# cvxgrp/pymde

Measured on AMD Instinct MI355X. Metric: edges/sec/iter (avg_distortion fwd+bwd), n=1M |E|=50M d=2, higher is better.
Workload: dtype f32; 1 GPU; BASELINE configs[3] / SURVEY 8d config 4a: n=1000000, |E|=50000000 uniform-random edges (out-degree 50), d=2, penalties.Log1p(1.5), weights in {1,2}; seeded on the device with torch.Generator(0) (the survey's recipe uses numpy default_rng(0): same distribution, another stream; --survey-seed builds that one); parallelism=single GPU, parameter_stream=codebook: 2 distinct weights ride in the packed half-edge word (4 B/half-edge)

## Files before the change

### include/mde_hip.h

```cpp
#ifndef MDE_HIP_H_
#define MDE_HIP_H_

#include <stdint.h>

#ifdef __cplusplus
extern "C" {
#endif

#define MDE_ABI_VERSION 2

#define MDE_OK 0
#define MDE_E_INVALID (-1)
#define MDE_E_SELF_EDGE (-2)
#define MDE_E_RANGE (-3)
#define MDE_E_TOO_LARGE (-4)
#define MDE_E_HIP (-5)
#define MDE_E_UNSUPPORTED (-6)

const char* mde_last_error(void);
int mde_abi_version(void);

enum {
  MDE_F_NONE = 0,
  MDE_F_LINEAR = 1,
// ... 59 lines not shown
int mde_shard_bounds(int64_t n, int64_t p, const int64_t* edges, int32_t world,
                     int64_t* bounds_host, void* stream);

int mde_plan_expand(const mde_plan* plan, const float* in_edge, float* out_half, void* stream);

int mde_plan_layout(mde_plan* plan, int32_t d, void* stream);
int mde_plan_function_hint(mde_plan* plan, int32_t kind, int32_t kind_neg);
int64_t mde_plan_layout_half_edges(const mde_plan* plan, int32_t layout);
int mde_plan_expand_codebook(const mde_plan* plan, const float* in_edge, float* out_half,
                             int32_t* n_values_host, void* stream);
int mde_plan_expand_bytes(const mde_plan* plan, const float* in_edge, float* out_half,
                          int32_t* n_values_host, void* stream);
int mde_plan_expand_layout(const mde_plan* plan, int32_t layout, const float* in_edge,
                           float* out_half, void* stream);
int mde_plan_ring_info(const mde_plan* plan, int64_t* info_host);
int mde_plan_ring_check(const mde_plan* plan, int64_t* out_host, void* stream);
int mde_plan_row_order(mde_plan* plan, int32_t mode, void* stream, double* info_host);
int mde_plan_loss_double(const mde_plan* plan, double* dst, void* stream);

int mde_edges_deduplicate(int64_t n, int64_t p, const int64_t* edges, int64_t* edges_out,
                          int64_t* count_host, void* stream);
int mde_edges_count_unique(int64_t n, int64_t p, const int64_t* edges, int64_t* edges_out,
                           float* weights_out, int64_t* count_host, void* stream);
int mde_knn(int64_t n, int32_t nf, const float* data, int32_t k, int32_t* idx_out, float* d2_out,
            float* sqn_work, void* stream);
int mde_row_sqnorm(int64_t n, int32_t nf, const float* data, float* out, void* stream);
int64_t mde_col_stats_work_bytes(int64_t n, int32_t nf);
int mde_col_stats(int64_t n, int32_t nf, const float* data, double* stats_out, int32_t* bad_row_out, void* work,
                  void* stream);
int mde_rows_subtract(int64_t n, int32_t nf, const float* data, const double* mu, float* out, void* stream);
// ... 193 lines not shown
```

### pymde_amd/_lib.py

```python
import ctypes
import os
import threading

import torch

_HERE = os.path.dirname(os.path.abspath(__file__))
LIB_PATH = os.path.join(_HERE, "libmde_hip.so")

c_i32, c_i64, c_f32 = ctypes.c_int32, ctypes.c_int64, ctypes.c_float
c_vp = ctypes.c_void_p

MDE_OK = 0
MDE_E_INVALID, MDE_E_SELF_EDGE, MDE_E_RANGE = -1, -2, -3
MDE_E_TOO_LARGE, MDE_E_HIP, MDE_E_UNSUPPORTED = -4, -5, -6


class MdeFunc(ctypes.Structure):
    _fields_ = [("kind", c_i32), ("kind_neg", c_i32), ("a0", c_vp), ("a1", c_vp),
                ("a0_scalar", c_i32), ("a1_scalar", c_i32),
                ("s0", c_f32), ("s1", c_f32), ("s2", c_f32),
                ("n0", c_f32), ("n1", c_f32), ("n2", c_f32), ("layout", c_i32),
                ("e0", c_vp), ("e1", c_vp)]


# ... 13 lines not shown
    "mde_plan_destroy": (c_i32, [c_vp]),
    "mde_plan_n": (c_i64, [c_vp]),
    "mde_plan_p": (c_i64, [c_vp]),
    "mde_plan_half_edges": (c_i64, [c_vp]),
    "mde_plan_row_lo": (c_i64, [c_vp]),
    "mde_plan_row_hi": (c_i64, [c_vp]),
    "mde_plan_rowptr": (c_vp, [c_vp]),
    "mde_plan_nbr": (c_vp, [c_vp]),
    "mde_plan_eid": (c_vp, [c_vp]),
    "mde_plan_export": (c_i32, [c_vp, c_vp, c_vp, c_vp, c_vp]),
    "mde_shard_bounds": (c_i32, [c_i64, c_i64, c_vp, c_i32, ctypes.POINTER(c_i64), c_vp]),
    "mde_plan_expand": (c_i32, [c_vp, c_vp, c_vp, c_vp]),
    "mde_plan_layout": (c_i32, [c_vp, c_i32, c_vp]),
    "mde_plan_layout_half_edges": (c_i64, [c_vp, c_i32]),
    "mde_plan_ring_info": (c_i32, [c_vp, ctypes.POINTER(c_i64)]),
    "mde_plan_ring_check": (c_i32, [c_vp, ctypes.POINTER(c_i64), c_vp]),
    "mde_plan_row_order": (c_i32, [c_vp, c_i32, c_vp, ctypes.POINTER(ctypes.c_double)]),
    "mde_plan_function_hint": (c_i32, [c_vp, c_i32, c_i32]),
    "mde_plan_loss_double": (c_i32, [c_vp, c_vp, c_vp]),
    "mde_center_step_begin": (c_i32, [c_i64, c_i32, c_vp, c_vp, c_f32, c_vp, c_vp, c_vp]),
    "mde_center_step_end": (c_i32, [c_i64, c_i32, c_vp, c_vp, ctypes.c_double, c_vp]),
    "mde_lbfgs_dev_stage": (c_i32, [c_vp, c_vp, c_vp, c_vp, c_f32, c_vp, c_vp]),
    "mde_lbfgs_dev_finish": (c_i32, [c_vp, c_vp, c_vp, c_vp, c_vp, c_vp]),
    "mde_lbfgs_dev_dots": (c_i32, [c_vp]),
    "mde_rank_reduce": (c_i32, [c_i32, c_i32, ctypes.c_uint64, c_vp, c_vp, c_i32, c_vp, c_vp]),
    "mde_plan_expand_codebook": (c_i32, [c_vp, c_vp, c_vp, ctypes.POINTER(c_i32), c_vp]),
    "mde_plan_expand_bytes": (c_i32, [c_vp, c_vp, c_vp, ctypes.POINTER(c_i32), c_vp]),
    "mde_plan_expand_layout": (c_i32, [c_vp, c_i32, c_vp, c_vp, c_vp]),
    "mde_edges_deduplicate": (c_i32, [c_i64, c_i64, c_vp, c_vp, ctypes.POINTER(c_i64), c_vp]),
    "mde_edges_count_unique": (c_i32, [c_i64, c_i64, c_vp, c_vp, c_vp, ctypes.POINTER(c_i64), c_vp]),
# ... 161 lines not shown
```

### pymde_amd/average_distortion.py

```python
import ctypes

import torch

from pymde_amd import _lib
from pymde_amd import util


def _check_X(X, n=None, d=None):
    if not isinstance(X, torch.Tensor) or X.dim() != 2:
        raise ValueError("the embedding must be a 2-D tensor")
    if X.dtype != torch.float32:
        raise ValueError(
            "pymde_amd computes in float32; got an embedding of dtype %s (MDE.embed and "
            "MDE.average_distortion cast float64 inputs with a warning; the kernels themselves do not)" % X.dtype)
    util.require_cuda_device(X.device)
    if n is not None and X.shape[0] != n:
        raise ValueError("embedding has %d rows, the problem has %d items" % (X.shape[0], n))


class EdgePlan(object):

    def __init__(self, n_items, edges, row_lo=0, row_hi=None):
        lib = _lib.load()
        device = util.require_cuda_device(edges.device)
# ... 61 lines not shown
        if t.numel() != self.p:
            return None
        size = int(lib.mde_plan_layout_half_edges(self._handle, 1))
        out = torch.empty(max(size, 1), dtype=torch.float32, device=self.device)
        nv = ctypes.c_int32(0)
        with torch.cuda.device(self.device):
            _lib.check(lib.mde_plan_expand_bytes(self._handle, _lib.ptr(t), _lib.ptr(out),
                                                 ctypes.byref(nv), _lib.stream_ptr(self.device)))
        return out if nv.value > 0 else None

    def ring_info(self):
        lib = _lib.load()
        info = (ctypes.c_int64 * 16)()
        _lib.check(lib.mde_plan_ring_info(self._handle, info))
        names = ("built", "d", "rows_per_block", "row_blocks", "col_groups", "chunks", "ring_slots", "iterations",
                 "ring_half_edges", "padded_entries", "permuted", "hub_rows", "hub_half_edges", "hub_segments")
        out = {k: int(info[i]) for i, k in enumerate(names)}
        out["built"], out["permuted"] = bool(out["built"]), bool(out["permuted"])
        return out

    def ring_check(self):
        lib = _lib.load()
        out = (ctypes.c_int64 * 3)()
        with torch.cuda.device(self.device):
            _lib.check(lib.mde_plan_ring_check(self._handle, out, _lib.stream_ptr(self.device)))
        return {"split": int(out[0]), "shared": int(out[1]), "pairs": int(out[2])}

    def row_order(self, mode=1):
        lib = _lib.load()
        info = (ctypes.c_double * 4)()
        with torch.cuda.device(self.device):
            _lib.check(lib.mde_plan_row_order(self._handle, int(mode), _lib.stream_ptr(self.device), info))
        return {"in_use": bool(info[0]), "mean_distance_before": float(info[1]),
                "mean_distance_after": float(info[2]), "levels": int(info[3])}

    def csr(self):
        lib = _lib.load()
        nloc = self.row_hi - self.row_lo
        rowptr = torch.empty(nloc + 1, dtype=torch.int32, device=self.device)
        nbr = torch.empty(max(self.half_edges, 1), dtype=torch.int32, device=self.device)
        eid = torch.empty(max(self.half_edges, 1), dtype=torch.int32, device=self.device)
# ... 224 lines not shown
```

### pymde_amd/csrc/mde_plan.h

```cpp
#pragma once
#include "mde_common.h"

struct mde_ring_layout {
  int d = 0;
  int rejected_d = 0;
  float cost_scale = 1.0f;
  int rows_per_block = 0, n_row_blocks = 0;
  int col_groups = 1;
  int chunk_cols = 0, n_chunks = 0;
  int ring_off = 0, slots = 0;
  int64_t n_iters = 0;
  int64_t H = 0;
  uint32_t* packed = nullptr;
  int32_t* eid = nullptr;
  uint32_t* hdr = nullptr;
  int32_t* wave_iter = nullptr;
  float* partial = nullptr;
  int32_t* slot_row = nullptr;
  int count_all = 0;
  int n_hub_rows = 0, n_hub_segs = 0;
  int64_t hub_half_edges = 0;
  int32_t* hub_rows = nullptr;
  int32_t* hub_seg = nullptr;
  int32_t* hub_first = nullptr;
  double* hub_partial = nullptr;
};
#define MDE_HUB_SEG 512

struct mde_plan {
  int64_t n = 0, p = 0, H = 0, row_lo = 0, row_hi = 0;
  int32_t* rowptr = nullptr;
  int32_t* nbr = nullptr;
  int32_t* eid = nullptr;
  double* partials = nullptr;
// ... 22 lines not shown
```

### pymde_amd/csrc/mde_ring.h

```cpp
#pragma once
#include "mde_common.h"
#include "mde_functions.h"
#include "mde_plan.h"

#define MDE_RING_LDS_BYTES 163840
__host__ __device__ constexpr int ring_row_cap(int d) { return d == 1 ? 12288 : (d == 2 ? 7816 : (d == 3 ? 5200 : 3936)); }
__host__ __device__ constexpr int ring_ctrl_off(int d) { return (ring_row_cap(d) + 32) * 4 * d; }
__host__ __device__ constexpr int ring_gr_off(int d) { return ring_ctrl_off(d) + 256; }
#define MDE_RING_CTRL_PROG(d) (ring_ctrl_off(d))
#define MDE_RING_CTRL_F(d) (ring_ctrl_off(d) + 64)
#define MDE_RING_CTRL_CB(d) (ring_ctrl_off(d) + 96)
#ifndef MDE_RING_NCW
#define MDE_RING_NCW 8
#endif
#ifndef MDE_RING_CSLEEP
#define MDE_RING_CSLEEP 1
#endif
#ifndef MDE_RING_PSLEEP
#define MDE_RING_PSLEEP 1
#endif
#ifndef MDE_RING_PRODPRIO
#define MDE_RING_PRODPRIO 2
#endif
#ifndef MDE_RING_CONSPRIO
// ... 39 lines not shown
#ifdef MDE_RING_SPAN
  return MDE_RING_SPAN;
#endif
  return S - 5 > 6 ? 6 : (S - 5 < 2 ? 2 : S - 5);
}

#define MDE_RING_HDR(m, span, rounds, pad) ((uint32_t)(m) | ((uint32_t)(span) << 16) | ((uint32_t)(rounds) << 21) | ((uint32_t)(pad) << 27))

#define MDE_RING_HW 4
#define MDE_RING_H3_PAD 4u

__host__ __device__ inline uint32_t ring_pack_word(int d, uint32_t rowaddr, uint32_t coladdr) {
  return d == 2 ? (rowaddr | ((coladdr >> 3) << 16)) : (rowaddr | ((coladdr >> 2) << 16));
}

struct RingArgs {
  mde_plan* plan;
  const float* X;
  int d;
  const float *a0, *a1;
  int a0_scalar, a1_scalar;
  float* grad;
  float inv_p, grad_scale;
  hipStream_t st;
  float* loss_out;
  double loss_scale;
};

inline MdeFuncArgs ring_func_args(const mde_func* f) {
  MdeFuncArgs a;
// ... 15 lines not shown
```

### pymde_amd/csrc/mde_ring.hip

```cpp
#include <algorithm>
#include <chrono>
#include <cmath>
#include <cstring>
#include <vector>

#include "mde_ring.h"

#ifndef MDE_RING_BUCKETS
#define MDE_RING_BUCKETS 32
#endif
__global__ __launch_bounds__(64) void k_ring_assign(int nloc, int R, int Q, int NC, int C, int contiguous,
                                                    const int32_t* __restrict__ rowptr,
                                                    const int32_t* __restrict__ nbr, uint32_t* __restrict__ wmap,
                                                    int32_t* __restrict__ wrows) {
  constexpr int B = MDE_RING_BUCKETS, NCWP = MDE_RING_NCW <= 8 ? 8 : 16, LPW = 64 / NCWP, BPL = B / LPW;
  static_assert(MDE_RING_NCW <= 16 && B % LPW == 0 && B <= 64, "lane map of k_ring_assign");
  __shared__ int hist[B];
  __shared__ float cpre[B];
  const int wg = blockIdx.x, rb = wg / Q, g = wg % Q, lane = threadIdx.x;
  const int j_lo = (int)(((int64_t)g * NC + Q - 1) / Q), j_hi = (int)(((int64_t)(g + 1) * NC + Q - 1) / Q);
  const int nj = max(1, j_hi - j_lo);
  const int r0 = rb * R, nr = min(R, nloc - r0);
  const int w = lane / LPW, bg = lane % LPW;
  uint32_t* out = wmap + (size_t)wg * R;
// ... 378 lines not shown
  }
  return half * 32 + quarter * 16 + pos;
}

__global__ __launch_bounds__(MDE_BLOCK) void k_ring_pack(int64_t nit, int nseg, const int32_t* __restrict__ iter_base,
                                                         const int32_t* __restrict__ src_base,
                                                         const int32_t* __restrict__ it_ent,
                                                         const int32_t* __restrict__ it_cnt,
                                                         const int32_t* __restrict__ it_m,
                                                         const uint32_t* __restrict__ keys,
                                                         const uint32_t* __restrict__ vals,
                                                         const int32_t* __restrict__ hrow,
                                                         const int32_t* __restrict__ nbr,
                                                         const int32_t* __restrict__ eid, int R, int Q, int C, int S,
                                                         int ring_off, int JB, int d, int row_lo, int place, int count_all,
                                                         uint32_t* __restrict__ packed,
                                                         int32_t* __restrict__ peid, uint32_t* __restrict__ hdr) {
  __shared__ uint8_t s_taken[MDE_BLOCK / 64][64], s_free[MDE_BLOCK / 64][64];
  __shared__ uint32_t s_prow[MDE_BLOCK / 64][64];
  const int lane = threadIdx.x & 63, wv = threadIdx.x >> 6;
  const int64_t nw = ((int64_t)gridDim.x * MDE_BLOCK) >> 6;
  const uint32_t JM = (1u << JB) - 1u;
  const int sh = ring_cls_shift(d), cm = ring_cls_mask(d);
  const uint32_t cbytes = (uint32_t)C * 4u * (uint32_t)d;
  for (int64_t itb = (int64_t)blockIdx.x * (MDE_BLOCK / 64); itb < nit; itb += nw) {
    const int64_t it = itb + wv;
    const bool valid = it < nit;
    int64_t src = it;
    if (valid && src_base) {
      int lo = 0, hi = nseg;
      while (hi - lo > 1) {
// ... 46 lines not shown
      }
    }
    __syncthreads();
    const bool moved = second && act && pin < 0 && s_taken[wv][l];
    if (second && act && !moved) s_taken[wv][l] = 1;
    __syncthreads();
    {
      const bool fr = !s_taken[wv][lane];
      const unsigned long long fm = __ballot(fr);
      if (fr) s_free[wv][__popcll(fm & ((1ull << lane) - 1ull))] = (uint8_t)lane;
    }
    __syncthreads();
    const unsigned long long mvm = __ballot(moved);
    const int nmoved = __popcll(mvm);
    if (moved) l = s_free[wv][__popcll(mvm & ((1ull << lane) - 1ull))];
    const bool counts = act && (count_all || (uint32_t)(row_lo + grow) < col);
    const int ncount = __popcll(__ballot(counts));
    const uint32_t lclass = ncount == 0 ? 0u : (ncount == cnt ? 1u : 2u);
    const uint32_t m = valid ? (uint32_t)__builtin_amdgcn_readfirstlane(it_m[src]) : 0u;
    const uint32_t need = max((uint32_t)(cw >> 8), m);
    const uint32_t mpad = valid ? (uint32_t)__builtin_amdgcn_readfirstlane(it_m[src & ~(int64_t)1]) : 0u;
    const size_t base = ((size_t)(it >> 2) * 64) * 4 + (size_t)(it & 3);
    if (act) {
      packed[base + (size_t)l * 4] = ring_pack_word(d, rowaddr, ring);
      peid[base + (size_t)l * 4] = eid[q];
    } else if (valid) {
      const int lf = s_free[wv][nmoved + lane - cnt];
      packed[base + (size_t)lf * 4] = ring_pack_word(d, (uint32_t)(R + (lf & 31)) * 4u * (uint32_t)d,
                                                     (uint32_t)ring_off + (mpad % (uint32_t)S) * cbytes);
      peid[base + (size_t)lf * 4] = -1;
    }
    if (lane == 0 && valid) {
      hdr[MDE_RING_HW * it] = m;
      hdr[MDE_RING_HW * it + 1] = need;
      hdr[MDE_RING_HW * it + 2] = lclass;
      hdr[MDE_RING_HW * it + 3] = (cnt < 64 ? MDE_RING_H3_PAD : 0u) | ((uint32_t)cnt << 8);
    }
    __syncthreads();
  }
}

__global__ __launch_bounds__(MDE_BLOCK) void k_ring_block_class(int64_t nblocks, uint32_t* __restrict__ hdr) {
  const int64_t b = (int64_t)blockIdx.x * MDE_BLOCK + threadIdx.x;
  if (b >= nblocks) return;
  bool any0 = false, any1 = false, any2 = false;
  for (int q = 0; q < 4; ++q) {
    const uint32_t* h = hdr + (size_t)MDE_RING_HW * (4 * b + q);
    if ((h[3] >> 8) == 0u) continue;
    any0 |= h[2] == 0u;
    any1 |= h[2] == 1u;
    any2 |= h[2] == 2u;
// ... 13 lines not shown
__global__ __launch_bounds__(MDE_BLOCK) void k_ring_stats(int64_t nit, const uint32_t* __restrict__ hdr,
                                                          unsigned long long* __restrict__ stats) {
  unsigned long long a = 0, b = 0, c = 0;
  for (int64_t i = (int64_t)blockIdx.x * MDE_BLOCK + threadIdx.x; i < nit; i += (int64_t)gridDim.x * MDE_BLOCK) {
    a += (hdr[MDE_RING_HW * i + 3] & MDE_RING_H3_PAD) ? 1u : 0u;
    b += hdr[MDE_RING_HW * i + 2] == 1u;
    c += hdr[MDE_RING_HW * i + 2] == 2u;
  }
  a = mde_wave_sum(a);
  b = mde_wave_sum(b);
  c = mde_wave_sum(c);
  if ((threadIdx.x & 63) == 0) {
    atomicAdd(&stats[0], a);
    atomicAdd(&stats[1], b);
    atomicAdd(&stats[2], c);
  }
}

__global__ __launch_bounds__(MDE_BLOCK) void k_ring_sweep_balance(int nwg, int ngroups, int GW, int JB,
                                                                  const uint32_t* __restrict__ keys,
                                                                  const int32_t* __restrict__ seg,
                                                                  unsigned long long* __restrict__ crit,
                                                                  unsigned long long* __restrict__ tot) {
  const int64_t idx = (int64_t)blockIdx.x * MDE_BLOCK + threadIdx.x;
  if (idx >= (int64_t)nwg * ngroups) return;
  const int wg = (int)(idx / ngroups), g = (int)(idx % ngroups);
  unsigned long long mx = 0, sm = 0;
  for (int w = 0; w < MDE_RING_NCW; ++w) {
    const uint32_t s = (uint32_t)wg * MDE_RING_NCW + (uint32_t)w;
    const int32_t lo = seg[s], hi = seg[s + 1];
// ... 574 lines not shown
  if (e == hipSuccess) e = hipMalloc(&peid, (size_t)Hp * sizeof(int32_t));
  if (e == hipSuccess) e = hipMalloc(&hdr, (size_t)total_iters * MDE_RING_HW * sizeof(uint32_t));
  const size_t partial_floats = (size_t)z.Q * (size_t)nloc * (size_t)d;
  if (e == hipSuccess && z.Q > 1) e = hipMalloc(&partial, sizeof(float) * (partial_floats + 2 * (size_t)z.NRB));
  if (e == hipSuccess && z.Q > 1) e = hipMemsetAsync(partial + partial_floats, 0, sizeof(float) * 2 * (size_t)z.NRB, st);
  if (e != hipSuccess) {
    drop_caps();
    return fail(e, "ring layout: output allocations");
  }
  tick("output allocations");
  if (!single) {
    hipLaunchKernelGGL(k_ring_schedule<true>, dim3(nseg), dim3(64), flag_bytes, st, nseg, seg, wrows, keys2, meta, JM, span, z.R,
                       z.Q, z.NC, d, cap, 0, nullptr, iter_base, it_ent, it_cnt, it_m, flag_rows, nullptr);
    e = hipGetLastError();
  }
  if (e == hipSuccess) {
    hipLaunchKernelGGL(k_ring_pack, dim3(mde_grid((int64_t)total_iters * 64, MDE_BLOCK, 8192)), dim3(MDE_BLOCK), 0, st,
                       (int64_t)total_iters, nseg, iter_base, single ? cap_base : nullptr, it_ent, it_cnt, it_m, keys2, vals2, hrow,
                       plan->nbr, plan->eid, z.R, z.Q, z.C, z.S, z.ring_off, z.JB, d, (int)plan->row_lo, place, rp.permuted ? 1 : 0,
                       packed, peid, hdr);
    e = hipGetLastError();
  }
  if (e == hipSuccess) e = hipStreamSynchronize(st);
  drop_caps();
  if (e != hipSuccess) return fail(e, "ring layout: fill / pack");
  hipLaunchKernelGGL(k_ring_block_class, dim3((unsigned)((total_iters / 4 + MDE_BLOCK - 1) / MDE_BLOCK)), dim3(MDE_BLOCK), 0, st,
                     (int64_t)(total_iters / 4), hdr);
  RB(hipGetLastError());
  RB(hipStreamSynchronize(st));
  if (getenv("MDE_RING_STATS")) {
    unsigned long long* dstat = reinterpret_cast<unsigned long long*>(iters);
    unsigned long long hstat[3] = {0, 0, 0};
    RB(hipMemsetAsync(dstat, 0, sizeof(hstat), st));
    hipLaunchKernelGGL(k_ring_stats, dim3(256), dim3(MDE_BLOCK), 0, st, (int64_t)total_iters, hdr, dstat);
    RB(hipMemcpyAsync(hstat, dstat, sizeof(hstat), hipMemcpyDeviceToHost, st));
    RB(hipStreamSynchronize(st));
    {
      std::vector<int32_t> hb((size_t)nseg + 1);
      RB(hipMemcpy(hb.data(), iter_base, hb.size() * sizeof(int32_t), hipMemcpyDeviceToHost));
      int mx = 0, mn = 1 << 30, wg_mx = 0;
      for (int i = 0; i < nseg; ++i) {
        mx = std::max(mx, hb[i + 1] - hb[i]);
        mn = std::min(mn, hb[i + 1] - hb[i]);
      }
// ... 63 lines not shown
  L.n_row_blocks = z.NRB;
  L.col_groups = z.Q;
  L.chunk_cols = z.C;
  L.n_chunks = z.NC;
  L.ring_off = z.ring_off;
  L.slots = z.S;
  L.n_iters = total_iters;
  L.H = Hp;
  L.packed = packed;
  L.eid = peid;
  L.hdr = hdr;
  L.wave_iter = iter_base;
  L.partial = partial;
  L.slot_row = slot_row;
  L.count_all = rp.permuted ? 1 : 0;
  L.n_hub_rows = (int)rp.hub_rows.size();
  L.n_hub_segs = (int)(rp.hub_seg.size() / 4);
  L.hub_half_edges = rp.hub_half_edges;
  L.hub_rows = hub_rows;
  L.hub_seg = hub_seg;
  L.hub_first = hub_first;
  L.hub_partial = hub_partial;
  return 1;
}

extern "C" int mde_plan_layout(mde_plan* plan, int32_t d, void* stream) {
  if (!plan || d <= 0) return MDE_E_INVALID;
  if (plan->ring.packed && plan->ring.d == d) return 1;
  RingSizes z;
  if (!choose_sizes(plan, d, &z)) return 0;
// ... 292 lines not shown
  if (!L.packed) return MDE_OK;
  info[0] = 1;
  info[1] = L.d;
  info[2] = L.rows_per_block;
  info[3] = L.n_row_blocks;
  info[4] = L.col_groups;
  info[5] = L.n_chunks;
  info[6] = L.slots;
  info[7] = L.n_iters;
  info[8] = plan->H - L.hub_half_edges;
  info[9] = L.H;
  info[10] = L.slot_row ? 1 : 0;
  info[11] = L.n_hub_rows;
  info[12] = L.hub_half_edges;
  info[13] = L.n_hub_segs;
  return MDE_OK;
}

__global__ __launch_bounds__(MDE_BLOCK) void k_ring_pair_check(int64_t npairs, const uint32_t* __restrict__ packed, int d, int R,
                                                               unsigned long long* __restrict__ out) {
  const int lane = threadIdx.x & 63;
  const int64_t nw = ((int64_t)gridDim.x * MDE_BLOCK) >> 6;
  const uint32_t mask = d == 2 ? 0xfff8u : 0xfffcu, dummy = (uint32_t)R * 4u * (uint32_t)d;
  unsigned long long split = 0, shared = 0, pairs = 0;
  for (int64_t pr = ((int64_t)blockIdx.x * MDE_BLOCK + threadIdx.x) >> 6; pr < npairs; pr += nw) {
    const int64_t it = 2 * pr;
    const size_t base = ((size_t)(it >> 2) * 64 + (size_t)lane) * 4 + (size_t)(it & 3);
    const uint32_t ra = packed[base] & mask, rb = packed[base + 1] & mask;
    int found = -1;
    for (int k = 0; k < 64; ++k)
      if ((uint32_t)__builtin_amdgcn_readlane((int)ra, k) == rb) found = k;
    const bool real = rb < dummy;
    split += __popcll(__ballot(real && found >= 0 && found != lane));
    shared += __popcll(__ballot(real && found >= 0));
    ++pairs;
  }
  if (lane == 0) {
    atomicAdd(&out[0], split);
    atomicAdd(&out[1], shared);
    atomicAdd(&out[2], pairs);
  }
}

extern "C" int mde_plan_ring_check(const mde_plan* plan, int64_t* out_host, void* stream) {
  if (!plan || !out_host) return MDE_E_INVALID;
  const mde_ring_layout& L = plan->ring;
  for (int i = 0; i < 3; ++i) out_host[i] = 0;
  if (!L.packed || L.n_iters == 0) return MDE_OK;
  hipStream_t st = mde_stream(stream);
  unsigned long long* dout = nullptr;
  hipError_t e = hipMalloc(&dout, 3 * sizeof(unsigned long long));
  if (e == hipSuccess) e = hipMemsetAsync(dout, 0, 3 * sizeof(unsigned long long), st);
  if (e == hipSuccess) {
    hipLaunchKernelGGL(k_ring_pair_check, dim3(mde_grid(L.n_iters / 2 * 64, MDE_BLOCK, 4096)), dim3(MDE_BLOCK), 0, st,
                       L.n_iters / 2, L.packed, L.d, L.rows_per_block, dout);
    e = hipGetLastError();
  }
  unsigned long long h[3] = {0, 0, 0};
  if (e == hipSuccess) e = hipMemcpyAsync(h, dout, sizeof(h), hipMemcpyDeviceToHost, st);
  if (e == hipSuccess) e = hipStreamSynchronize(st);
  if (dout) (void)hipFree(dout);
  if (e != hipSuccess) {
    mde_set_error("mde_plan_ring_check: %s", hipGetErrorString(e));
    return MDE_E_HIP;
  }
  for (int i = 0; i < 3; ++i) out_host[i] = (int64_t)h[i];
  return MDE_OK;
}

extern "C" int mde_plan_expand_layout(const mde_plan* plan, int32_t layout, const float* in_edge,
                                      float* out_half, void* stream) {
  if (!plan || !in_edge || !out_half) return MDE_E_INVALID;
  if (layout == 0) return mde_plan_expand(plan, in_edge, out_half, stream);
  if (layout != 1 || !plan->ring.eid) {
    mde_set_error("mde_plan_expand_layout: the LDS-ring layout has not been built");
    return MDE_E_INVALID;
  }
  if (plan->ring.H == 0) return MDE_OK;
  hipLaunchKernelGGL(k_expand_ring, dim3(mde_grid(plan->ring.H, MDE_BLOCK, 4096)), dim3(MDE_BLOCK), 0,
                     mde_stream(stream), plan->ring.H, plan->ring.eid, in_edge, out_half);
  MDE_LAUNCH_CHECK();
  return MDE_OK;
}

template <int D>
__global__ __launch_bounds__(MDE_BLOCK) void k_hub_rows(const int32_t* __restrict__ hub_rows, const int32_t* __restrict__ hub_seg,
                                                        int row_lo, const int32_t* __restrict__ nbr,
                                                        const int32_t* __restrict__ eid, const float* __restrict__ e0,
                                                        const float* __restrict__ e1, int e0_scalar, int e1_scalar,
                                                        const float* __restrict__ X, FnRuntime fn, float inv_p, int count_all,
                                                        double* __restrict__ partial) {
  __shared__ double smem[8];
  const int sgi = blockIdx.x;
  const int hi = hub_seg[4 * sgi], beg = hub_seg[4 * sgi + 1], end = hub_seg[4 * sgi + 2];
  const int64_t v = (int64_t)row_lo + hub_rows[hi];
  float xv[D];
#pragma unroll
  for (int c = 0; c < D; ++c) xv[c] = X[v * D + c];
  const float e0s = e0_scalar ? e0[0] : 0.0f;
  const float e1s = (e1 && e1_scalar) ? e1[0] : 0.0f;
  double acc[D], loss = 0.0;
#pragma unroll
  for (int c = 0; c < D; ++c) acc[c] = 0.0;
  for (int h = beg + (int)threadIdx.x; h < end; h += MDE_BLOCK) {
    const int u = nbr[h], k = eid[h];
    const float p0 = e0_scalar ? e0s : e0[k];
    const float p1 = (e1 && !e1_scalar) ? e1[k] : e1s;
    float diff[D], ss = 0.0f;
#pragma unroll
    for (int c = 0; c < D; ++c) {
      diff[c] = xv[c] - X[(size_t)u * D + c];
      ss = fmaf(diff[c], diff[c], ss);
    }
    float f, gd;
    fn.eval(ss, p0, p1, f, gd);
    const float g = mde_fix_g(gd * inv_p);
    if (count_all || v < (int64_t)u) loss += (double)f;
#pragma unroll
    for (int c = 0; c < D; ++c) acc[c] += (double)(g * diff[c]);
  }
#pragma unroll
  for (int c = 0; c < D; ++c) {
    const double t = mde_block_sum(acc[c], smem);
    if (threadIdx.x == 0) partial[(size_t)sgi * 8 + c] = t;
  }
  const double tl = mde_block_sum(loss, smem);
  if (threadIdx.x == 0) partial[(size_t)sgi * 8 + 4] = tl;
}

template <int D>
__global__ __launch_bounds__(64) void k_hub_finish(int n_hub, int n_seg, const int32_t* __restrict__ hub_rows,
                                                   const int32_t* __restrict__ hub_first,
// ... 23 lines not shown
  double t = 0.0;
  for (int sg = lane; sg < n_seg; sg += 64) t += partial[(size_t)sg * 8 + 4];
  const double tot = mde_wave_sum(t);
  if (lane == 0) {
    *loss_d += tot * loss_scale;
    *loss_out = (float)*loss_d;
  }
}

template <int D>
static int hub_launch_d(const mde_plan* plan, const float* X, const mde_func* f, const float* e0, const float* e1, int e0_scalar,
                        int e1_scalar, float grad_scale, float* grad, float inv_p, hipStream_t st, float* loss_out, double loss_scale) {
  const mde_ring_layout& L = plan->ring;
  FnRuntime fn{ring_func_args(f)};
  hipLaunchKernelGGL(k_hub_rows<D>, dim3(L.n_hub_segs), dim3(MDE_BLOCK), 0, st, L.hub_rows, L.hub_seg, (int)plan->row_lo, plan->nbr,
                     plan->eid, e0, e1, e0_scalar, e1_scalar, X, fn, inv_p, L.count_all, L.hub_partial);
  MDE_LAUNCH_CHECK();
  const int nb = L.n_hub_rows + 1;
  hipLaunchKernelGGL(k_hub_finish<D>, dim3(nb), dim3(64), 0, st, L.n_hub_rows, L.n_hub_segs, L.hub_rows, L.hub_first,
                     L.hub_partial, (int)plan->row_lo, grad_scale, grad, (L.count_all ? 1.0 : 2.0) * loss_scale, loss_out,
                     plan->partials + MDE_PARTIALS_LOSS_D);
  MDE_LAUNCH_CHECK();
  return MDE_OK;
}

static int hub_launch(const mde_plan* plan, const float* X, int d, const mde_func* f, float grad_scale, float* grad, float inv_p,
                      hipStream_t st, float* loss_out, double loss_scale) {
  const float *e0 = f->e0, *e1 = f->e1;
  int e0_scalar = 0, e1_scalar = 0;
  if (f->a0_scalar == 1) {
    e0 = f->a0;
// ... 49 lines not shown
```

### pymde_amd/csrc/mde_ring_kernel.h

```cpp
#pragma once
#include <algorithm>
#include <cstring>
#include <type_traits>
#include <vector>

#include "mde_ring.h"
#define COMMA ,

#define MDE_RING23(FN, LIN)                                    \
  do {                                                         \
    FN fn{a};                                                  \
    int rc;                                                    \
    if (A.d == 2)                                              \
      rc = launch_ring<2, FN, LIN>(A, fn, nblocks);            \
    else                                                       \
      rc = launch_ring<3, FN, LIN>(A, fn, nblocks);            \
    return rc == MDE_OK ? 1 : rc;                              \
  } while (0)

typedef uint32_t ring_u4 __attribute__((ext_vector_type(4)));
typedef float ring_f4 __attribute__((ext_vector_type(4)));

template <int D>
struct RingVec;
// ... 396 lines not shown
        if constexpr (BX)
          r.p0 = *reinterpret_cast<const float*>(L + tab_off + bi4);
        else
          r.p0 = CB ? *reinterpret_cast<const float*>(L + CTRL_CB + ((w & (D == 2 ? 7u : 3u)) << 2)) : p0 * Fn::kParamScale;
#ifdef MDE_RING_KEEPROW
        r.row = row_of(w);
        ring_ld_operand<D>(L, r.row, r.xr);
#else
        ring_ld_operand<D>(L, row_of(w), r.xr);
#endif
        ring_ld_operand<D>(L, col_of(w), r.xc);
        return r;
      };
      auto bx4 = [&](uint32_t bw, int q) __attribute__((always_inline)) { return BX ? ((bw >> (8 * q)) & 0xffu) << 2 : 0u; };
      auto counts_here = [&](uint32_t w, uint32_t hm) __attribute__((always_inline)) {
        const uint32_t off = col_of(w) - (uint32_t)ring_off;
        const uint32_t slot = off / (uint32_t)CBYTES, cidx = (off - slot * (uint32_t)CBYTES) / (4u * (uint32_t)D);
        const uint32_t ms = hm % (uint32_t)S;
        const uint32_t j = hm + (slot >= ms ? slot - ms : slot + (uint32_t)S - ms);
        const uint32_t u = j * (uint32_t)C + cidx;
        const uint32_t vv = (uint32_t)(row_lo + r0) + row_of(w) / (4u * (uint32_t)D);
        return vv < u;
      };
      auto finish = [&](auto lc_tag, uint32_t w, const Pre& x, float (&acc)[D], float p1, uint32_t hm)
          __attribute__((always_inline)) {
        constexpr int LC = decltype(lc_tag)::value;
#ifdef MDE_RING_KEEPROW
        const uint32_t rowaddr = x.row;
#else
        const uint32_t rowaddr = row_of(w);
#endif
        float v[D], ss = (defined_MDE_RING_EVAL2 && Fn::kRingFused) ? 1.0e-30f : 0.0f;
#pragma unroll
        for (int c = 0; c < D; ++c) {
          v[c] = x.xr[c] - x.xc[c];
          ss = fmaf(v[c], v[c], ss);
        }
// ... 106 lines not shown

      Pre xa, xb;
      float acc[D], accb[D];
      auto block_body = [&](auto lc_tag, int u, int b) __attribute__((always_inline)) {
#pragma unroll
        for (int h = 0; h < 2; ++h) {
          const int q = 2 * h;
          const int un = h == 0 ? u : (u + 1) % PFB, qn = (q + 2) & 3;
          wait_pair(un, qn);
          const Pre xna = issue_x(pq[un][qn], (a0_scalar || PS != 0) ? a0s : wq[un][qn], bx4(bq[un], qn));
          const Pre xnb = issue_x(pq[un][qn + 1], (a0_scalar || PS != 0) ? a0s : wq[un][qn + 1], bx4(bq[un], qn + 1));
          release_to((u + 1) % PFB, q);
          prefetch_landed();
          const float p1a = a1_arr ? a1[((size_t)((ib >> 2) + b) * 64 + lane) * 4 + q] : a1s;
          const float p1b = a1_arr ? a1[((size_t)((ib >> 2) + b) * 64 + lane) * 4 + q + 1] : a1s;
          const bool lc2 = decltype(lc_tag)::value == 2;
          const uint32_t hma = lc2 ? (uint32_t)__builtin_amdgcn_readlane((int)hv[u], 4 * q) : 0u;
          const uint32_t hmb = lc2 ? (uint32_t)__builtin_amdgcn_readlane((int)hv[u], 4 * q + 4) : 0u;
          finish(lc_tag, pq[u][q], xa, acc, p1a, hma);
          if (HAS_GRAD) {
            const bool same = row_of(pq[u][q + 1]) == row_of(pq[u][q]);
#pragma unroll
            for (int c = 0; c < D; ++c) accb[c] = same ? acc[c] : accb[c];
          }
          finish(lc_tag, pq[u][q + 1], xb, accb, p1b, hmb);
          if (HAS_GRAD) {
            ring_ld<D>(L + GR_OFF + row_of(pq[un][qn]), acc);
            ring_ld<D>(L + GR_OFF + row_of(pq[un][qn + 1]), accb);
          }
          xa = xna;
          xb = xnb;
// ... 352 lines not shown
```

Before: 317.3 billion edges/s/iter.

## Precompute loss-ownership bit in packed word and band-balance loss ownership

```diff
diff --git a/include/mde_hip.h b/include/mde_hip.h
--- a/include/mde_hip.h
+++ b/include/mde_hip.h
@@ -97,6 +97,7 @@
 int mde_plan_expand_layout(const mde_plan* plan, int32_t layout, const float* in_edge,
                            float* out_half, void* stream);
 int mde_plan_ring_info(const mde_plan* plan, int64_t* info_host);
+int mde_plan_ring_loss_balance(const mde_plan* plan, double* out_host);
 int mde_plan_ring_check(const mde_plan* plan, int64_t* out_host, void* stream);
 int mde_plan_row_order(mde_plan* plan, int32_t mode, void* stream, double* info_host);
 int mde_plan_loss_double(const mde_plan* plan, double* dst, void* stream);
diff --git a/pymde_amd/_lib.py b/pymde_amd/_lib.py
--- a/pymde_amd/_lib.py
+++ b/pymde_amd/_lib.py
@@ -51,6 +51,7 @@
     "mde_plan_layout": (c_i32, [c_vp, c_i32, c_vp]),
     "mde_plan_layout_half_edges": (c_i64, [c_vp, c_i32]),
     "mde_plan_ring_info": (c_i32, [c_vp, ctypes.POINTER(c_i64)]),
+    "mde_plan_ring_loss_balance": (c_i32, [c_vp, ctypes.POINTER(ctypes.c_double)]),
     "mde_plan_ring_check": (c_i32, [c_vp, ctypes.POINTER(c_i64), c_vp]),
     "mde_plan_row_order": (c_i32, [c_vp, c_i32, c_vp, ctypes.POINTER(ctypes.c_double)]),
     "mde_plan_function_hint": (c_i32, [c_vp, c_i32, c_i32]),
diff --git a/pymde_amd/average_distortion.py b/pymde_amd/average_distortion.py
--- a/pymde_amd/average_distortion.py
+++ b/pymde_amd/average_distortion.py
@@ -99,17 +99,22 @@
         info = (ctypes.c_int64 * 16)()
         _lib.check(lib.mde_plan_ring_info(self._handle, info))
         names = ("built", "d", "rows_per_block", "row_blocks", "col_groups", "chunks", "ring_slots", "iterations",
-                 "ring_half_edges", "padded_entries", "permuted", "hub_rows", "hub_half_edges", "hub_segments")
+                 "ring_half_edges", "padded_entries", "permuted", "hub_rows", "hub_half_edges", "hub_segments", "loss_band")
         out = {k: int(info[i]) for i, k in enumerate(names)}
         out["built"], out["permuted"] = bool(out["built"]), bool(out["permuted"])
+        bal = (ctypes.c_double * 8)()
+        _lib.check(lib.mde_plan_ring_loss_balance(self._handle, bal))
+        out["class_blocks"] = tuple(int(bal[i]) for i in (1, 2, 3))
+        out["loss_share_min"], out["loss_share_max"] = float(bal[4]), float(bal[5])
         return out
 
     def ring_check(self):
         lib = _lib.load()
-        out = (ctypes.c_int64 * 3)()
+        out = (ctypes.c_int64 * 8)()
         with torch.cuda.device(self.device):
             _lib.check(lib.mde_plan_ring_check(self._handle, out, _lib.stream_ptr(self.device)))
-        return {"split": int(out[0]), "shared": int(out[1]), "pairs": int(out[2])}
+        return {"split": int(out[0]), "shared": int(out[1]), "pairs": int(out[2]), "loss_bad": int(out[3]),
+                "loss_flag_bad": int(out[4]), "loss_edges": int(out[5])}
 
     def row_order(self, mode=1):
         lib = _lib.load()
diff --git a/pymde_amd/csrc/mde_plan.h b/pymde_amd/csrc/mde_plan.h
--- a/pymde_amd/csrc/mde_plan.h
+++ b/pymde_amd/csrc/mde_plan.h
@@ -18,6 +18,9 @@
   float* partial = nullptr;
   int32_t* slot_row = nullptr;
   int count_all = 0;
+  int loss_band = 0;
+  int64_t class_blocks[3] = {0, 0, 0};
+  double loss_share_min = 0.0, loss_share_max = 0.0;
   int n_hub_rows = 0, n_hub_segs = 0;
   int64_t hub_half_edges = 0;
   int32_t* hub_rows = nullptr;
diff --git a/pymde_amd/csrc/mde_ring.h b/pymde_amd/csrc/mde_ring.h
--- a/pymde_amd/csrc/mde_ring.h
+++ b/pymde_amd/csrc/mde_ring.h
@@ -77,6 +77,13 @@
   return d == 2 ? (rowaddr | ((coladdr >> 3) << 16)) : (rowaddr | ((coladdr >> 2) << 16));
 }
 
+#define MDE_RING_COUNTS_BIT 0x80000000u
+
+__host__ __device__ inline bool ring_counts(uint32_t v, uint32_t u, uint32_t W) {
+  const bool lower = v < u;
+  return W ? (lower != (((v / W + u / W) & 1u) != 0u)) : lower;
+}
+
 struct RingArgs {
   mde_plan* plan;
   const float* X;
diff --git a/pymde_amd/csrc/mde_ring.hip b/pymde_amd/csrc/mde_ring.hip
--- a/pymde_amd/csrc/mde_ring.hip
+++ b/pymde_amd/csrc/mde_ring.hip
@@ -416,7 +416,7 @@
                                                          const int32_t* __restrict__ nbr,
                                                          const int32_t* __restrict__ eid, int R, int Q, int C, int S,
                                                          int ring_off, int JB, int d, int row_lo, int place, int count_all,
-                                                         uint32_t* __restrict__ packed,
+                                                         int loss_band, uint32_t* __restrict__ packed,
                                                          int32_t* __restrict__ peid, uint32_t* __restrict__ hdr) {
   __shared__ uint8_t s_taken[MDE_BLOCK / 64][64], s_free[MDE_BLOCK / 64][64];
   __shared__ uint32_t s_prow[MDE_BLOCK / 64][64];
@@ -493,7 +493,7 @@
     const unsigned long long mvm = __ballot(moved);
     const int nmoved = __popcll(mvm);
     if (moved) l = s_free[wv][__popcll(mvm & ((1ull << lane) - 1ull))];
-    const bool counts = act && (count_all || (uint32_t)(row_lo + grow) < col);
+    const bool counts = act && (count_all || ring_counts((uint32_t)(row_lo + grow), col, (uint32_t)loss_band));
     const int ncount = __popcll(__ballot(counts));
     const uint32_t lclass = ncount == 0 ? 0u : (ncount == cnt ? 1u : 2u);
     const uint32_t m = valid ? (uint32_t)__builtin_amdgcn_readfirstlane(it_m[src]) : 0u;
@@ -501,7 +501,7 @@
     const uint32_t mpad = valid ? (uint32_t)__builtin_amdgcn_readfirstlane(it_m[src & ~(int64_t)1]) : 0u;
     const size_t base = ((size_t)(it >> 2) * 64) * 4 + (size_t)(it & 3);
     if (act) {
-      packed[base + (size_t)l * 4] = ring_pack_word(d, rowaddr, ring);
+      packed[base + (size_t)l * 4] = ring_pack_word(d, rowaddr, ring) | ((d == 2 && counts) ? MDE_RING_COUNTS_BIT : 0u);
       peid[base + (size_t)l * 4] = eid[q];
     } else if (valid) {
       const int lf = s_free[wv][nmoved + lane - cnt];
@@ -513,7 +513,7 @@
       hdr[MDE_RING_HW * it] = m;
       hdr[MDE_RING_HW * it + 1] = need;
       hdr[MDE_RING_HW * it + 2] = lclass;
-      hdr[MDE_RING_HW * it + 3] = (cnt < 64 ? MDE_RING_H3_PAD : 0u) | ((uint32_t)cnt << 8);
+      hdr[MDE_RING_HW * it + 3] = (cnt < 64 ? MDE_RING_H3_PAD : 0u) | ((uint32_t)cnt << 8) | ((uint32_t)ncount << 16);
     }
     __syncthreads();
   }
@@ -557,6 +557,35 @@
     atomicAdd(&stats[0], a);
     atomicAdd(&stats[1], b);
     atomicAdd(&stats[2], c);
+  }
+}
+
+__global__ __launch_bounds__(64) void k_ring_loss_stats(const int32_t* __restrict__ wave_iter, const uint32_t* __restrict__ hdr,
+                                                        unsigned long long* __restrict__ wg, unsigned long long* __restrict__ cls) {
+  const int g = blockIdx.x, lane = threadIdx.x;
+  const int64_t i0 = wave_iter[(size_t)g * MDE_RING_NCW], i1 = wave_iter[(size_t)(g + 1) * MDE_RING_NCW];
+  unsigned long long ent = 0, cnt = 0, c0 = 0, c1 = 0, c2 = 0;
+  for (int64_t i = i0 + lane; i < i1; i += 64) {
+    const uint32_t h3 = hdr[MDE_RING_HW * i + 3];
+    ent += (h3 >> 8) & 0xffu;
+    cnt += (h3 >> 16) & 0xffu;
+    if ((i & 3) == 0) {
+      c0 += (h3 & 3u) == 0u;
+      c1 += (h3 & 3u) == 1u;
+      c2 += (h3 & 3u) == 2u;
+    }
+  }
+  ent = mde_wave_sum(ent);
+  cnt = mde_wave_sum(cnt);
+  c0 = mde_wave_sum(c0);
+  c1 = mde_wave_sum(c1);
+  c2 = mde_wave_sum(c2);
+  if (lane == 0) {
+    wg[2 * g] = ent;
+    wg[2 * g + 1] = cnt;
+    atomicAdd(&cls[0], c0);
+    atomicAdd(&cls[1], c1);
+    atomicAdd(&cls[2], c2);
   }
 }
 
@@ -1161,11 +1190,17 @@
                        z.Q, z.NC, d, cap, 0, nullptr, iter_base, it_ent, it_cnt, it_m, flag_rows, nullptr);
     e = hipGetLastError();
   }
+  int loss_band = 0;
+  if (d == 2 && !rp.permuted && plan->row_lo == 0 && nloc == plan->n) {
+    int64_t wb = std::max<int64_t>(1, (int64_t)z.NRB / (8 * (int64_t)z.Q));
+    if (getenv("MDE_RING_LOSS_BAND")) wb = std::max(0, atoi(getenv("MDE_RING_LOSS_BAND")));
+    loss_band = (int)std::min<int64_t>(wb * (int64_t)z.R, (int64_t)1 << 30);
+  }
   if (e == hipSuccess) {
     hipLaunchKernelGGL(k_ring_pack, dim3(mde_grid((int64_t)total_iters * 64, MDE_BLOCK, 8192)), dim3(MDE_BLOCK), 0, st,
                        (int64_t)total_iters, nseg, iter_base, single ? cap_base : nullptr, it_ent, it_cnt, it_m, keys2, vals2, hrow,
                        plan->nbr, plan->eid, z.R, z.Q, z.C, z.S, z.ring_off, z.JB, d, (int)plan->row_lo, place, rp.permuted ? 1 : 0,
-                       packed, peid, hdr);
+                       loss_band, packed, peid, hdr);
     e = hipGetLastError();
   }
   if (e == hipSuccess) e = hipStreamSynchronize(st);
@@ -1175,6 +1210,22 @@
                      (int64_t)(total_iters / 4), hdr);
   RB(hipGetLastError());
   RB(hipStreamSynchronize(st));
+  const int nwg = z.NRB * z.Q;
+  std::vector<unsigned long long> lstat((size_t)2 * nwg + 3, 0ull);
+  {
+    unsigned long long* dl = nullptr;
+    const size_t lb = lstat.size() * sizeof(unsigned long long);
+    e = hipMalloc(&dl, lb);
+    if (e == hipSuccess) e = hipMemsetAsync(dl, 0, lb, st);
+    if (e == hipSuccess) {
+      hipLaunchKernelGGL(k_ring_loss_stats, dim3(nwg), dim3(64), 0, st, iter_base, hdr, dl, dl + 2 * (size_t)nwg);
+      e = hipGetLastError();
+    }
+    if (e == hipSuccess) e = hipMemcpyAsync(lstat.data(), dl, lb, hipMemcpyDeviceToHost, st);
+    if (e == hipSuccess) e = hipStreamSynchronize(st);
+    if (dl) (void)hipFree(dl);
+    if (e != hipSuccess) return fail(e, "ring layout: loss statistics");
+  }
   if (getenv("MDE_RING_STATS")) {
     unsigned long long* dstat = reinterpret_cast<unsigned long long*>(iters);
     unsigned long long hstat[3] = {0, 0, 0};
@@ -1268,6 +1319,19 @@
   L.partial = partial;
   L.slot_row = slot_row;
   L.count_all = rp.permuted ? 1 : 0;
+  L.loss_band = loss_band;
+  {
+    double lo = 2.0, hi = -1.0;
+    for (int g = 0; g < nwg; ++g) {
+      if (lstat[2 * (size_t)g] == 0) continue;
+      const double sh = (double)lstat[2 * (size_t)g + 1] / (double)lstat[2 * (size_t)g];
+      lo = std::min(lo, sh);
+      hi = std::max(hi, sh);
+    }
+    L.loss_share_min = hi < 0.0 ? 0.0 : lo;
+    L.loss_share_max = hi < 0.0 ? 0.0 : hi;
+    for (int c = 0; c < 3; ++c) L.class_blocks[c] = (int64_t)lstat[2 * (size_t)nwg + c];
+  }
   L.n_hub_rows = (int)rp.hub_rows.size();
   L.n_hub_segs = (int)(rp.hub_seg.size() / 4);
   L.hub_half_edges = rp.hub_half_edges;
@@ -1590,6 +1654,19 @@
   info[11] = L.n_hub_rows;
   info[12] = L.hub_half_edges;
   info[13] = L.n_hub_segs;
+  info[14] = L.loss_band;
+  return MDE_OK;
+}
+
+extern "C" int mde_plan_ring_loss_balance(const mde_plan* plan, double* out) {
+  if (!plan || !out) return MDE_E_INVALID;
+  const mde_ring_layout& L = plan->ring;
+  for (int i = 0; i < 8; ++i) out[i] = 0.0;
+  if (!L.packed) return MDE_OK;
+  out[0] = (double)L.loss_band;
+  for (int c = 0; c < 3; ++c) out[1 + c] = (double)L.class_blocks[c];
+  out[4] = L.loss_share_min;
+  out[5] = L.loss_share_max;
   return MDE_OK;
 }
 
@@ -1618,29 +1695,122 @@
   }
 }
 
+__global__ __launch_bounds__(MDE_BLOCK) void k_ring_loss_mark(int64_t nit, int nseg, const int32_t* __restrict__ wave_iter,
+                                                              const uint32_t* __restrict__ hdr, const uint32_t* __restrict__ packed,
+                                                              const int32_t* __restrict__ peid, int d, int R, int Q, int C, int S,
+                                                              int ring_off, int row_lo, int loss_band, int64_t p,
+                                                              uint32_t* __restrict__ hist, unsigned long long* __restrict__ out) {
+  const int lane = threadIdx.x & 63;
+  const int64_t nw = ((int64_t)gridDim.x * MDE_BLOCK) >> 6;
+  const uint32_t cbytes = (uint32_t)C * 4u * (uint32_t)d;
+  unsigned long long mism = 0;
+  for (int64_t it = ((int64_t)blockIdx.x * MDE_BLOCK + threadIdx.x) >> 6; it < nit; it += nw) {
+    int lo = 0, hi = nseg;
+    while (hi - lo > 1) {
+      const int mid = (lo + hi) >> 1;
+      if ((int64_t)wave_iter[mid] <= it) lo = mid; else hi = mid;
+    }
+    const int rb = (lo / MDE_RING_NCW) / Q;
+    const size_t idx = ((size_t)(it >> 2) * 64 + (size_t)lane) * 4 + (size_t)(it & 3);
+    const uint32_t w = packed[idx];
+    const int32_t e = peid[idx];
+    const bool bit = d == 2 && (w & MDE_RING_COUNTS_BIT) != 0u;
+    if (e < 0 || (int64_t)e >= p) {
+      mism += bit ? 1u : 0u;
+      continue;
+    }
+    const uint32_t hm = hdr[MDE_RING_HW * it];
+    const uint32_t bcls = hdr[MDE_RING_HW * (it & ~(int64_t)3) + 3] & 3u;
+    const uint32_t rowaddr = d == 2 ? (w & 0xfff8u) : (w & 0xfffcu);
+    const uint32_t coladdr = d == 2 ? ((w >> 13) & 0x3fff8u) : ((w >> 14) & 0x3fffcu);
+    const uint32_t off = coladdr - (uint32_t)ring_off;
+    const uint32_t slot = off / cbytes, cidx = (off - slot * cbytes) / (4u * (uint32_t)d);
+    const uint32_t ms = hm % (uint32_t)S;
+    const uint32_t j = hm + (slot >= ms ? slot - ms : slot + (uint32_t)S - ms);
+    const uint32_t u = j * (uint32_t)C + cidx;
+    const uint32_t v = (uint32_t)row_lo + (uint32_t)rb * (uint32_t)R + rowaddr / (4u * (uint32_t)d);
+    const bool rule = ring_counts(v, u, (uint32_t)loss_band);
+    if (d == 2 && bit != rule) ++mism;
+    const bool here = bcls == 0u ? false : (bcls == 1u ? true : (d == 2 ? bit : rule));
+    atomicAdd(&hist[e], 0x10000u + (here ? 1u : 0u));
+  }
+  mism = mde_wave_sum(mism);
+  if (lane == 0 && mism) atomicAdd(&out[4], mism);
+}
+
+__global__ __launch_bounds__(MDE_BLOCK) void k_ring_loss_mark_hub(const int32_t* __restrict__ hub_rows, const int32_t* __restrict__ hub_seg,
+                                                                  int row_lo, const int32_t* __restrict__ nbr,
+                                                                  const int32_t* __restrict__ eid, int loss_band, int64_t p,
+                                                                  uint32_t* __restrict__ hist) {
+  const int sgi = blockIdx.x;
+  const int hi = hub_seg[4 * sgi], beg = hub_seg[4 * sgi + 1], end = hub_seg[4 * sgi + 2];
+  const uint32_t v = (uint32_t)row_lo + (uint32_t)hub_rows[hi];
+  for (int h = beg + (int)threadIdx.x; h < end; h += MDE_BLOCK) {
+    const int32_t e = eid[h];
+    if (e < 0 || (int64_t)e >= p) continue;
+    atomicAdd(&hist[e], 0x10000u + (ring_counts(v, (uint32_t)nbr[h], (uint32_t)loss_band) ? 1u : 0u));
+  }
+}
+
+__global__ __launch_bounds__(MDE_BLOCK) void k_ring_loss_count(int64_t p, const uint32_t* __restrict__ hist,
+                                                               unsigned long long* __restrict__ out) {
+  unsigned long long bad = 0, both = 0;
+  for (int64_t e = (int64_t)blockIdx.x * MDE_BLOCK + threadIdx.x; e < p; e += (int64_t)gridDim.x * MDE_BLOCK) {
+    const uint32_t seen = hist[e] >> 16, c = hist[e] & 0xffffu;
+    both += seen == 2u;
+    bad += seen > 2u || (seen == 2u && c != 1u) || (seen == 1u && c > 1u);
+  }
+  bad = mde_wave_sum(bad);
+  both = mde_wave_sum(both);
+  if ((threadIdx.x & 63) == 0) {
+    if (bad) atomicAdd(&out[3], bad);
+    if (both) atomicAdd(&out[5], both);
+  }
+}
+
 extern "C" int mde_plan_ring_check(const mde_plan* plan, int64_t* out_host, void* stream) {
   if (!plan || !out_host) return MDE_E_INVALID;
   const mde_ring_layout& L = plan->ring;
-  for (int i = 0; i < 3; ++i) out_host[i] = 0;
+  for (int i = 0; i < 8; ++i) out_host[i] = 0;
   if (!L.packed || L.n_iters == 0) return MDE_OK;
   hipStream_t st = mde_stream(stream);
   unsigned long long* dout = nullptr;
-  hipError_t e = hipMalloc(&dout, 3 * sizeof(unsigned long long));
-  if (e == hipSuccess) e = hipMemsetAsync(dout, 0, 3 * sizeof(unsigned long long), st);
+  uint32_t* hist = nullptr;
+  const bool loss_check = !L.count_all && plan->p > 0;
+  hipError_t e = hipMalloc(&dout, 8 * sizeof(unsigned long long));
+  if (e == hipSuccess) e = hipMemsetAsync(dout, 0, 8 * sizeof(unsigned long long), st);
   if (e == hipSuccess) {
     hipLaunchKernelGGL(k_ring_pair_check, dim3(mde_grid(L.n_iters / 2 * 64, MDE_BLOCK, 4096)), dim3(MDE_BLOCK), 0, st,
                        L.n_iters / 2, L.packed, L.d, L.rows_per_block, dout);
     e = hipGetLastError();
   }
-  unsigned long long h[3] = {0, 0, 0};
+  if (e == hipSuccess && loss_check) e = hipMalloc(&hist, (size_t)plan->p * sizeof(uint32_t));
+  if (e == hipSuccess && loss_check) e = hipMemsetAsync(hist, 0, (size_t)plan->p * sizeof(uint32_t), st);
+  if (e == hipSuccess && loss_check) {
+    hipLaunchKernelGGL(k_ring_loss_mark, dim3(mde_grid(L.n_iters * 64, MDE_BLOCK, 8192)), dim3(MDE_BLOCK), 0, st, L.n_iters,
+                       L.n_row_blocks * L.col_groups * MDE_RING_NCW, L.wave_iter, L.hdr, L.packed, L.eid, L.d, L.rows_per_block,
+                       L.col_groups, L.chunk_cols, L.slots, L.ring_off, (int)plan->row_lo, L.loss_band, plan->p, hist, dout);
+    e = hipGetLastError();
+  }
+  if (e == hipSuccess && loss_check && L.n_hub_segs > 0) {
+    hipLaunchKernelGGL(k_ring_loss_mark_hub, dim3(L.n_hub_segs), dim3(MDE_BLOCK), 0, st, L.hub_rows, L.hub_seg, (int)plan->row_lo,
+                       plan->nbr, plan->eid, L.loss_band, plan->p, hist);
+    e = hipGetLastError();
+  }
+  if (e == hipSuccess && loss_check) {
+    hipLaunchKernelGGL(k_ring_loss_count, dim3(mde_grid(plan->p, MDE_BLOCK, 4096)), dim3(MDE_BLOCK), 0, st, plan->p, hist, dout);
+    e = hipGetLastError();
+  }
+  unsigned long long h[8] = {0, 0, 0, 0, 0, 0, 0, 0};
   if (e == hipSuccess) e = hipMemcpyAsync(h, dout, sizeof(h), hipMemcpyDeviceToHost, st);
   if (e == hipSuccess) e = hipStreamSynchronize(st);
   if (dout) (void)hipFree(dout);
+  if (hist) (void)hipFree(hist);
   if (e != hipSuccess) {
     mde_set_error("mde_plan_ring_check: %s", hipGetErrorString(e));
     return MDE_E_HIP;
   }
-  for (int i = 0; i < 3; ++i) out_host[i] = (int64_t)h[i];
+  for (int i = 0; i < 8; ++i) out_host[i] = (int64_t)h[i];
   return MDE_OK;
 }
 
@@ -1665,7 +1835,7 @@
                                                         const int32_t* __restrict__ eid, const float* __restrict__ e0,
                                                         const float* __restrict__ e1, int e0_scalar, int e1_scalar,
                                                         const float* __restrict__ X, FnRuntime fn, float inv_p, int count_all,
-                                                        double* __restrict__ partial) {
+                                                        int loss_band, double* __restrict__ partial) {
   __shared__ double smem[8];
   const int sgi = blockIdx.x;
   const int hi = hub_seg[4 * sgi], beg = hub_seg[4 * sgi + 1], end = hub_seg[4 * sgi + 2];
@@ -1691,7 +1861,7 @@
     float f, gd;
     fn.eval(ss, p0, p1, f, gd);
     const float g = mde_fix_g(gd * inv_p);
-    if (count_all || v < (int64_t)u) loss += (double)f;
+    if (count_all || ring_counts((uint32_t)v, (uint32_t)u, (uint32_t)loss_band)) loss += (double)f;
 #pragma unroll
     for (int c = 0; c < D; ++c) acc[c] += (double)(g * diff[c]);
   }
@@ -1745,7 +1915,7 @@
   const mde_ring_layout& L = plan->ring;
   FnRuntime fn{ring_func_args(f)};
   hipLaunchKernelGGL(k_hub_rows<D>, dim3(L.n_hub_segs), dim3(MDE_BLOCK), 0, st, L.hub_rows, L.hub_seg, (int)plan->row_lo, plan->nbr,
-                     plan->eid, e0, e1, e0_scalar, e1_scalar, X, fn, inv_p, L.count_all, L.hub_partial);
+                     plan->eid, e0, e1, e0_scalar, e1_scalar, X, fn, inv_p, L.count_all, L.loss_band, L.hub_partial);
   MDE_LAUNCH_CHECK();
   const int nb = L.n_hub_rows + 1;
   hipLaunchKernelGGL(k_hub_finish<D>, dim3(nb), dim3(64), 0, st, L.n_hub_rows, L.n_hub_segs, L.hub_rows, L.hub_first,
diff --git a/pymde_amd/csrc/mde_ring_kernel.h b/pymde_amd/csrc/mde_ring_kernel.h
--- a/pymde_amd/csrc/mde_ring_kernel.h
+++ b/pymde_amd/csrc/mde_ring_kernel.h
@@ -434,13 +434,17 @@
       };
       auto bx4 = [&](uint32_t bw, int q) __attribute__((always_inline)) { return BX ? ((bw >> (8 * q)) & 0xffu) << 2 : 0u; };
       auto counts_here = [&](uint32_t w, uint32_t hm) __attribute__((always_inline)) {
-        const uint32_t off = col_of(w) - (uint32_t)ring_off;
-        const uint32_t slot = off / (uint32_t)CBYTES, cidx = (off - slot * (uint32_t)CBYTES) / (4u * (uint32_t)D);
-        const uint32_t ms = hm % (uint32_t)S;
-        const uint32_t j = hm + (slot >= ms ? slot - ms : slot + (uint32_t)S - ms);
-        const uint32_t u = j * (uint32_t)C + cidx;
-        const uint32_t vv = (uint32_t)(row_lo + r0) + row_of(w) / (4u * (uint32_t)D);
-        return vv < u;
+        if constexpr (D == 2) {
+          return (int)w < 0;
+        } else {
+          const uint32_t off = col_of(w) - (uint32_t)ring_off;
+          const uint32_t slot = off / (uint32_t)CBYTES, cidx = (off - slot * (uint32_t)CBYTES) / (4u * (uint32_t)D);
+          const uint32_t ms = hm % (uint32_t)S;
+          const uint32_t j = hm + (slot >= ms ? slot - ms : slot + (uint32_t)S - ms);
+          const uint32_t u = j * (uint32_t)C + cidx;
+          const uint32_t vv = (uint32_t)(row_lo + r0) + row_of(w) / (4u * (uint32_t)D);
+          return vv < u;
+        }
       };
       auto finish = [&](auto lc_tag, uint32_t w, const Pre& x, float (&acc)[D], float p1, uint32_t hm)
           __attribute__((always_inline)) {
@@ -577,7 +581,7 @@
           prefetch_landed();
           const float p1a = a1_arr ? a1[((size_t)((ib >> 2) + b) * 64 + lane) * 4 + q] : a1s;
           const float p1b = a1_arr ? a1[((size_t)((ib >> 2) + b) * 64 + lane) * 4 + q + 1] : a1s;
-          const bool lc2 = decltype(lc_tag)::value == 2;
+          const bool lc2 = decltype(lc_tag)::value == 2 && D != 2;
           const uint32_t hma = lc2 ? (uint32_t)__builtin_amdgcn_readlane((int)hv[u], 4 * q) : 0u;
           const uint32_t hmb = lc2 ? (uint32_t)__builtin_amdgcn_readlane((int)hv[u], 4 * q + 4) : 0u;
           finish(lc_tag, pq[u][q], xa, acc, p1a, hma);
```

Measured after the change: 320.7 billion edges/s/iter (median of 6 runs). 1.01x the previous value.
